# wirrell/SPART-python

Hardware: AMD Instinct MI355X
Metric: SPART spectra/sec (R_TOC+R_TOA+L_TOA) at batch 1M; achieved HBM GB/s vs peak (higher is better)
Workload: dtype f32

## Files before the change

spart-python_amd/build.py:

```python
import hashlib
import os
import subprocess
import sys
import tempfile

HERE = os.path.dirname(os.path.abspath(__file__))
CSRC = os.path.join(HERE, "csrc")
SRC = os.path.join(CSRC, "spart_capi.hip")
SOURCES = [SRC, os.path.join(CSRC, "spart_bands_f32.hip")]
DEPS = SOURCES + [os.path.join(CSRC, f) for f in ("spart_kernels.h", "spart_math.h", "spart_e3_coeffs.h", "spart_f64_tables.h",
                                                  "spart_bands_f32.h", "spart_lut.h")] + [os.path.join(HERE, "..", "include", "spart_hip.h")]
OUT = os.path.join(HERE, "libspart_hip.so")
CFLAGS = ["-O3", "--offload-arch=gfx950", "-std=c++17", "-fPIC", "-fno-slp-vectorize"]
LDFLAGS = ["--offload-arch=gfx950", "-shared", "-fPIC", "-ldl"]
FLAGS = CFLAGS + LDFLAGS
TU_FLAGS = {"spart_bands_f32.hip": ["-mllvm", "-amdgpu-sched-strategy=iterative-minreg"]}


def hipcc():
    for c in (os.environ.get("HIPCC"), "/opt/rocm/bin/hipcc", "hipcc"):
        if c and (os.path.isabs(c) and os.path.exists(c) or not os.path.isabs(c)):
            return c
    return "hipcc"


BUILD_ID_TAG = b"SPART_BUILD_ID:"


def tu_flags(src, extra=()):
    return CFLAGS + TU_FLAGS.get(os.path.basename(src), []) + list(extra)


def source_id(fast_math=True, extra=()):
    h = hashlib.sha256()
    for d in sorted(DEPS, key=os.path.basename):
        h.update(os.path.basename(d).encode() + b"\0")
        h.update(open(d, "rb").read())
    for s in SOURCES:
        h.update((os.path.basename(s) + ":" + " ".join(tu_flags(s, extra))).encode())
    h.update(" ".join(LDFLAGS).encode() + (b"|fast" if fast_math else b"|ieee"))
    return h.hexdigest()[:12]


def binary_id(path=None):
    try:
        data = open(path or OUT, "rb").read()
    except OSError:
        return None
    i = data.find(BUILD_ID_TAG)
    if i < 0:
        return None
    j = i + len(BUILD_ID_TAG)
    return data[j:j + 12].decode("ascii", "replace")


def needs_build(fast_math=True):
    return binary_id() != source_id(fast_math)


def device_asm(outdir, extra=()):
    outs, procs = [], []
    for s in SOURCES:
        o = os.path.join(outdir, os.path.basename(s) + ".s")
        procs.append(subprocess.Popen([hipcc(), *tu_flags(s, extra), "-DSPART_FAST_MATH=1", "-S", "--cuda-device-only", "-o", o, s],
                                      stderr=subprocess.DEVNULL))
        outs.append(o)
    for p in procs:
        if p.wait() != 0:
            raise subprocess.CalledProcessError(p.returncode, p.args)
    return outs


def _compile_and_link(out, defines, extra, verbose):
    with tempfile.TemporaryDirectory(prefix="spart_build_") as tmp:
        objs, procs = [], []
        for s in SOURCES:
            o = os.path.join(tmp, os.path.basename(s) + ".o")
            cmd = [hipcc(), *tu_flags(s, extra), *defines, "-c", "-o", o, s]
            if verbose:
                print("[spart_amd] " + " ".join(cmd), file=sys.stderr, flush=True)
            procs.append((subprocess.Popen(cmd), cmd))
            objs.append(o)
        for p, cmd in procs:
            if p.wait() != 0:
                raise subprocess.CalledProcessError(p.returncode, cmd)
        cmd = [hipcc(), *LDFLAGS, "-o", out, *objs]
        if verbose:
            print("[spart_amd] " + " ".join(cmd), file=sys.stderr, flush=True)
        subprocess.check_call(cmd)


def build(force=False, fast_math=None, verbose=True, out=None, extra=()):
    if out is not None:
        _compile_and_link(out, ["-DSPART_FAST_MATH=1", f'-DSPART_BUILD_ID="{source_id(True, extra)}"'], extra, verbose)
        return out
    if fast_math is None:
        fast_math = os.environ.get("SPART_FAST_MATH", "1") == "1"
    if not force and not needs_build(fast_math):
        return OUT
    tmp = f"{OUT}.tmp.{os.getpid()}"
    defines = [f'-DSPART_BUILD_ID="{source_id(fast_math)}"'] + (["-DSPART_FAST_MATH=1"] if fast_math else [])
    try:
        _compile_and_link(tmp, defines, (), verbose)
        os.replace(tmp, OUT)
    finally:
        if os.path.exists(tmp):
            os.remove(tmp)
    return OUT


if __name__ == "__main__":
    build(force="--force" in sys.argv, fast_math=True if "--fast-math" in sys.argv else None)
    print(OUT)
```

spart-python_amd/csrc/spart_kernels.h:

```cpp
#pragma once

#include "spart_math.h"

namespace spart {

constexpr int TILE = 256;
constexpr int NTILE = 8;
constexpr int NTILE_FULL = 9;
constexpr int MAX_NB = NWLS;

__device__ __forceinline__ void xcd_map(unsigned b, int& tile, int64_t& ck) {
  tile = (int)((b >> 3) & 7u);
  ck = (int64_t)(b >> 6) * 8 + (b & 7u);
}
inline unsigned xcd_grid(int64_t nchunk) { return (unsigned)(((nchunk + 7) / 8) * 64); }

struct ParamPtrs {
  const double* p[NPARAM];
  const double* rho_th;
  const double* tau_th;
  const double* lidf;
  int nlayers;
};

inline int64_t row_pitch_of(int64_t B) { return (B + 63) & ~int64_t(63); }

template <typename T> struct ConstCol {
  const T* p;
  int64_t stride;
  __device__ __forceinline__ T operator[](int i) const { return p[(int64_t)i * stride]; }
};

template <typename T>
__device__ __forceinline__ void stage_constants(T* lds_c, const T* __restrict__ blk, int64_t Bp, int nsub) {
  static_assert(TILE == 256 && NCONST % 8 == 0, "8 rows of 32 samples per pass");
  const int si = threadIdx.x & 31, i0 = threadIdx.x >> 5;
  const unsigned lane_off = ((unsigned)i0 * (unsigned)Bp + (unsigned)si) * (unsigned)sizeof(T);
  if (si < nsub) {
#pragma unroll
    for (int k = 0; k < NCONST / 8; ++k) {
      const T* row = blk + (int64_t)(8 * k) * Bp;
      lds_c[si * NCONST + i0 + 8 * k] = *reinterpret_cast<const T*>(reinterpret_cast<const char*>(row) + lane_off);
    }
  }
}

template <typename T, int SUB>
__device__ __forceinline__ void stage_fetch(T (&r)[NCONST * SUB / TILE], const T* __restrict__ blk, int64_t Bp, int nsub) {
  constexpr int RP = TILE / SUB;
  static_assert(TILE % SUB == 0 && NCONST % RP == 0, "whole passes");
  const int si = threadIdx.x % SUB, i0 = threadIdx.x / SUB;
  const unsigned lane_off = ((unsigned)i0 * (unsigned)Bp + (unsigned)si) * (unsigned)sizeof(T);
  if (si < nsub) {
#pragma unroll
    for (int k = 0; k < NCONST / RP; ++k) {
      const T* row = blk + (int64_t)(RP * k) * Bp;
      r[k] = *reinterpret_cast<const T*>(reinterpret_cast<const char*>(row) + lane_off);
    }
  }
}
template <typename T, int SUB>
__device__ __forceinline__ void stage_put(T* lds_c, const T (&r)[NCONST * SUB / TILE], int nsub) {
  constexpr int RP = TILE / SUB;
  const int si = threadIdx.x % SUB, i0 = threadIdx.x / SUB;
  if (si < nsub) {
#pragma unroll
    for (int k = 0; k < NCONST / RP; ++k) lds_c[si * NCONST + i0 + RP * k] = r[k];
  }
}

struct PreludeStore {
  float* cstF;
  double* cstD;
  double* atm;
  int64_t Bp, s;
  __device__ __forceinline__ void c(int i, double v) const {
    if (cstF) cstF[i * Bp + s] = (float)v;
    if (cstD) cstD[i * Bp + s] = v;
  }
  __device__ __forceinline__ void a(int i, double v) const {
    if (atm) atm[i * Bp + s] = v;
  }
  __device__ __forceinline__ void l(int, double) const {}
};

constexpr int PRELUDE_SIMD_WAVES = 3;
template <bool FAST, bool USER = false>
__global__ __launch_bounds__(256, PRELUDE_SIMD_WAVES) void k_prelude(ParamPtrs pp, int mask, int64_t B, int64_t Bp, float* __restrict__ cstF,
                                                 double* __restrict__ cstD, double* __restrict__ atm) {
  const int64_t base = (int64_t)blockIdx.x * blockDim.x;
  int64_t s = base + threadIdx.x;
  if (!FAST && (mask & PRE_CANOPY) && !(USER && pp.lidf)) {
    constexpr int NB = 32;
    __shared__ int cnt[NB], start[NB];
    __shared__ unsigned char perm[256];
    const int t = threadIdx.x;
    int bucket = NB - 1;
    if (s < B) {
      const double key = ::fabs(pp.p[16][s]) + ::fabs(pp.p[17][s]);
      const double q = key * (NB / 1.0);
      bucket = !(q < (double)(NB - 1)) ? NB - 1 : (q > 0.0 ? (int)q : 0);
    }
    if (t < NB) cnt[t] = 0;
    __syncthreads();
    const int pos = atomicAdd(&cnt[bucket], 1);
    __syncthreads();
    if (t == 0) {
      int acc = 0;
      for (int i = 0; i < NB; ++i) { start[i] = acc; acc += cnt[i]; }
    }
    __syncthreads();
    perm[start[bucket] + pos] = (unsigned char)t;
    __syncthreads();
    s = base + perm[t];
  }
  if (s >= B) return;
  double rho_th = pp.rho_th ? pp.rho_th[s] : 0.01;
  double tau_th = pp.tau_th ? pp.tau_th[s] : 0.01;
  PreludeStore out{cstF, cstD, atm, Bp, s};
  if (USER)
    sample_prelude_to<FAST, true>([&pp, s](int i) { return pp.p[i] ? pp.p[i][s] : 0.0; }, rho_th, tau_th, mask, out,
                                  pp.lidf ? pp.lidf + s * NLINCL : nullptr, pp.nlayers);
  else
    sample_prelude_to<FAST>([&pp, s](int i) { return pp.p[i] ? pp.p[i][s] : 0.0; }, rho_th, tau_th, mask, out);
}

static __global__ __launch_bounds__(256) void k_lidf(const double* __restrict__ a, const double* __restrict__ b, int64_t B,
                                              double* __restrict__ lidf) {
  int64_t s = (int64_t)blockIdx.x * blockDim.x + threadIdx.x;
  if (s >= B) return;
  double li[NLINCL];
  leaf_angles(a[s], b[s], li);
#pragma unroll
  for (int i = 0; i < NLINCL; ++i) lidf[s * NLINCL + i] = li[i];
}

template <typename T> __device__ __forceinline__ BandTab<T> load_tab(const T* __restrict__ tab, int i) {
  BandTab<T> t;
  t.kab = tab[TAB_KAB * NWL + i];
  t.kca = tab[TAB_KCA * NWL + i];
  t.kdm = tab[TAB_KDM * NWL + i];
  t.kw = tab[TAB_KW * NWL + i];
  t.ks = tab[TAB_KS * NWL + i];
  t.kant = tab[TAB_KANT * NWL + i];
  t.kcbc = tab[TAB_CBC * NWL + i];
  t.kprot = tab[TAB_PROT * NWL + i];
  t.talf = tab[TAB_TALF * NWL + i];
  t.t12 = tab[TAB_T12 * NWL + i];
  t.t21 = tab[TAB_T21 * NWL + i];
  t.g0 = tab[TAB_GSV0 * NWL + i];
  t.g1 = tab[TAB_GSV1 * NWL + i];
  t.g2 = tab[TAB_GSV2 * NWL + i];
  t.cbac = tab[TAB_CBAC * NWL + i];
  t.pw = tab[TAB_PW * NWL + i];
  t.rw = tab[TAB_RW * NWL + i];
  return t;
}

template <typename T, typename C> __device__ __forceinline__ CanopyPar<T> load_canopy(const C& c) {
  CanopyPar<T> cp;
  cp.sob = c[C_SOB]; cp.sof = c[C_SOF];
  cp.hbf = c[C_HBF]; cp.ks = c[C_KS]; cp.ko = c[C_KO]; cp.lai = c[C_LAI]; cp.lai2 = c[C_LAI2];
  cp.tss = c[C_TSS]; cp.too = c[C_TOO]; cp.Z = c[C_Z]; cp.hot = c[C_HOT]; cp.pso2w = c[C_PSO2W];
  return cp;
}

template <bool NT = false, typename T> __device__ __forceinline__ void store_row(T* row, unsigned byte_off, T v) {
  T* p = reinterpret_cast<T*>(reinterpret_cast<char*>(row) + byte_off);
  if (NT) __builtin_nontemporal_store(v, p);
  else *p = v;
}
inline bool nt_ok(int pitch_elems, size_t elem_size) { return ((size_t)pitch_elems * elem_size) % 128 == 0; }

template <typename T> struct MatPtrs {
  T *leaf_refl, *leaf_tran, *leaf_kchl, *soil_refl, *soil_dry, *rso, *rdo, *rsd, *rdd;
  const T* rdry_in;
  int pf, po;
};

template <typename T, int MAT, int FULL, bool NT = false>
__global__ __launch_bounds__(TILE, (sizeof(T) == 8 ? 3 : 1))
void k_bands(const T* __restrict__ tab, const T* __restrict__ cst, int64_t Bp, int64_t B, int chunk, MatPtrs<T> mat,
             T* __restrict__ bandsum) {
  int tile;
  int64_t ck;
  xcd_map(blockIdx.x, tile, ck);
  if (ck * chunk >= B) return;
  if (sizeof(T) == 8) stage_f64_tables();
  const int band = tile * TILE + threadIdx.x;
  const bool active = band < NEVAL;
  const bool thermal = band == NWL;
  const int ti = band < NWL ? band : NWL - 1;
  const BandTab<T> tb = load_tab(tab, ti);
  const int64_t s0 = ck * chunk;
  const int64_t s1 = (s0 + chunk < B) ? s0 + chunk : B;
  T sum_so = T(0), sum_do = T(0), sum_sd = T(0), sum_dd = T(0);
  unsigned off_f = (unsigned)band * (unsigned)sizeof(T), off_o = off_f;
  if (MAT) {
    const int64_t b0f = s0 * mat.pf, b0o = s0 * mat.po;
    if (mat.leaf_refl) mat.leaf_refl += b0f;
    if (mat.leaf_tran) mat.leaf_tran += b0f;
    if (mat.soil_refl) mat.soil_refl += b0f;
    if (mat.rso) mat.rso += b0f;
    if (mat.rdo) mat.rdo += b0f;
    if (mat.rsd) mat.rsd += b0f;
    if (mat.rdd) mat.rdd += b0f;
    if (mat.leaf_kchl) mat.leaf_kchl += b0o;
    if (mat.soil_dry) mat.soil_dry += b0o;
  }
  constexpr int SUB = 32;
  constexpr bool HOIST_FILM = sizeof(T) == 8;
  constexpr bool PINGPONG = sizeof(T) == 4 && MAT == 0;
  __shared__ __attribute__((aligned(16))) T lds_all[(PINGPONG ? 2 : 1) * SUB * NCONST];
  T stg[NCONST * SUB / TILE];
  int cur = 0;
  if (PINGPONG) {
    const int n0 = (int)((s1 - s0 < SUB) ? (s1 - s0) : SUB);
    stage_fetch<T, SUB>(stg, cst + s0, Bp, n0);
    stage_put<T, SUB>(lds_all, stg, n0);
    __syncthreads();
  }
  for (int64_t sb = s0; sb < s1; sb += SUB) {
  const int nsub = (int)((s1 - sb < SUB) ? (s1 - sb) : SUB);
  T* const lds_c = lds_all + cur * (SUB * NCONST);
  const int nnext = (int)((s1 - sb - SUB < SUB) ? (s1 - sb - SUB) : SUB);
  if (PINGPONG) {
    if (nnext > 0) stage_fetch<T, SUB>(stg, cst + sb + SUB, Bp, nnext);
  } else {
    __syncthreads();
    stage_constants<T>(lds_c, cst + sb, Bp, nsub);
    __syncthreads();
  }
  bool film_same = false;
  T tw1s = T(0);
  if (HOIST_FILM) {
    const int l = threadIdx.x & 63;
    const T f0 = lds_c[C_FILM2L];
    const T fl = lds_c[(l < nsub ? l : 0) * NCONST + C_FILM2L];
    film_same = __all(fl == f0) != 0;
    if (film_same) tw1s = soil_tw1<T>(tb, f0);
  }
  constexpr bool AHEAD = MAT == 0 && sizeof(T) == 4;
  T lc[9];
#pragma unroll
  for (int i = 0; i < 9; ++i) lc[i] = lds_c[i];
  for (int si = 0; si < nsub; ++si) {
    const int64_t s = sb + si;
    const T* c = lds_c + si * NCONST;
    T refl, tran, absb, K;
    static_assert(C_CAB == 0 && C_NM1 == 8, "lc[] = constants 0..8 in leaf_band's argument order");
    if (!AHEAD) {
#pragma unroll
      for (int i = 0; i < 9; ++i) lc[i] = c[i];
    }
    leaf_band<T>(tb, lc[0], lc[1], lc[2], lc[3], lc[4], lc[5], lc[6], lc[7], lc[8], refl, tran, absb, K);
    if (AHEAD) {
      const T* cn = lds_c + ((si + 1 < nsub) ? si + 1 : si) * NCONST;
#pragma unroll
      for (int i = 0; i < 9; ++i) lc[i] = cn[i];
    }
    T rho = refl, tau = tran, ab = absb;
    if (tile == NTILE - 1) {
      rho = thermal ? c[C_RHO_TH] : refl;
      tau = thermal ? c[C_TAU_TH] : tran;
      ab = thermal ? (T(1) - c[C_RHO_TH] - c[C_TAU_TH]) : absb;
    }
    if (MAT && active) {
      if (mat.leaf_refl) store_row<NT>(mat.leaf_refl, off_f, rho);
      if (mat.leaf_tran) store_row<NT>(mat.leaf_tran, off_f, tau);
      if (!thermal && mat.leaf_kchl) store_row<NT>(mat.leaf_kchl, off_o, (K > T(0)) ? divx(c[C_CAB] * tb.kab, K) : T(0));
    }
    const CanopyPar<T> cp = load_canopy<T>(c);
    const CanopyCore<T> core = canopy_core_l<T>(cp, rho, tau, ab, c[C_KSL], c[C_KOL]);
    T rdry = (MAT == 2) ? mat.rdry_in[s * mat.po + ti] : soil_dry<T>(tb, c[C_F1], c[C_F2], c[C_F3]);
    T fm[7] = {c[C_FM0], c[C_FM1], c[C_FM2], c[C_FM3], c[C_FM4], c[C_FM5], c[C_FM6]};
    T rwet;
    if (HOIST_FILM) {
      const T tw1 = film_same ? tw1s : soil_tw1<T>(tb, c[C_FILM2L]);
      soil_band_tw<T>(tb, rdry, c[C_WET], fm, c[C_FMSUM], tw1, rwet);
    } else {
      soil_band<T>(tb, rdry, c[C_WET], fm, c[C_FMSUM], c[C_FILM2L], rwet);
    }
    if (MAT && active) {
      if (mat.soil_refl) store_row<NT>(mat.soil_refl, off_f, rwet);
      if (!thermal && mat.soil_dry) store_row<NT>(mat.soil_dry, off_o, rdry);
    }
    constexpr bool SUM_ONLY = FULL == 1 && MAT == 0 && sizeof(T) == 4;
    T rso, rdo, rsd, rdd;
    if (SUM_ONLY) {
      sum_so += canopy_soil_sum<T>(cp, core, rwet, c[C_TSTO]);
    } else {
      canopy_soil<T>(cp, core, rwet, rso, rdo, rsd, rdd);
      if (FULL == 2) {
        sum_so += rso; sum_do += rdo; sum_sd += rsd; sum_dd += rdd;
      } else if (FULL == 1) {
        sum_so += (rso + rdo) + (rsd + rdd);
      }
    }
    if (MAT) {
      if (active) {
        if (mat.rso) store_row<NT>(mat.rso, off_f, rso);
        if (mat.rdo) store_row<NT>(mat.rdo, off_f, rdo);
        if (mat.rsd) store_row<NT>(mat.rsd, off_f, rsd);
        if (mat.rdd) store_row<NT>(mat.rdd, off_f, rdd);
      }
      constexpr int TH_WAVE = (NWL % TILE) / 64, TH_LANE = (NWL % TILE) % 64;
      if (tile == NTILE - 1 && (int)(threadIdx.x >> 6) == TH_WAVE) {
        const unsigned pad = off_f + (unsigned)((TH_LANE + 1) * (int)sizeof(T));
        T* arrs[7] = {mat.leaf_refl, mat.leaf_tran, mat.soil_refl, mat.rso, mat.rdo, mat.rsd, mat.rdd};
        const T vals[7] = {rho, tau, rwet, rso, rdo, rsd, rdd};
        const int l = threadIdx.x & 63;
#pragma unroll
        for (int q = 0; q < 7; ++q) {
          const T v = __shfl(vals[q], TH_LANE, 64);
          if (arrs[q]) {
            store_row(arrs[q], pad, v);
            store_row(arrs[q], pad + 64u * (unsigned)sizeof(T), v);
            if (l < NWLT - 1 - 128) store_row(arrs[q], pad + 128u * (unsigned)sizeof(T), v);
          }
        }
      }
      off_f += (unsigned)mat.pf * (unsigned)sizeof(T);
      off_o += (unsigned)mat.po * (unsigned)sizeof(T);
    }
  }
  if (PINGPONG) {
    if (nnext > 0) stage_put<T, SUB>(lds_all + (cur ^ 1) * (SUB * NCONST), stg, nnext);
    __syncthreads();
    cur ^= 1;
  }
  }
  if (FULL == 2) {
    T* bs = bandsum + (ck * (NTILE * TILE) + band) * 4;
    bs[0] = sum_so; bs[1] = sum_do; bs[2] = sum_sd; bs[3] = sum_dd;
  } else if (FULL == 1) {
    bandsum[ck * (NTILE * TILE) + band] = sum_so;
  }
}

template <typename T> struct LdsCol {
  const T* p;
  __device__ __forceinline__ T operator[](int i) const { return p[i * 64]; }
};


constexpr int COL_WAVES = 4;
constexpr int COLUMNS_SIMD_WAVES = 4;

template <typename TG, typename TO, typename TR>
__global__ __launch_bounds__(64 * COL_WAVES, COLUMNS_SIMD_WAVES) void k_columns(
    const TG* __restrict__ tab, const TG* __restrict__ cst, const double* __restrict__ atm, int64_t Bp,
    const int* __restrict__ band0, const int* __restrict__ band1, const double* __restrict__ frac,
    const double* __restrict__ coef, const double* __restrict__ econv, int nb, const TR* __restrict__ rdry_in, int po, int64_t B,
    TO* __restrict__ R_TOC, TO* __restrict__ R_TOA, TO* __restrict__ L_TOA, TO* __restrict__ o_rsoil, TO* __restrict__ o_La) {
  __shared__ TG lds_c[NCONST_USED * 64];
  __shared__ double lds_a[NATM_USED * 64];
  __shared__ double lds_k[COL_WAVES * 64];
  if (sizeof(TG) == 8) stage_f64_tables();
  const int lane = threadIdx.x & 63;
  const int wave = __builtin_amdgcn_readfirstlane((int)(threadIdx.x >> 6));
  const int64_t s0 = (int64_t)blockIdx.x * 64;
  const int64_t s = s0 + lane;
  const bool ok = s < B;
  const int64_t sc = ok ? s : B - 1;
  for (int i = wave; i < NCONST_USED; i += COL_WAVES) lds_c[i * 64 + lane] = cst[(int64_t)i * Bp + sc];
  for (int i = wave; i < NATM_USED; i += COL_WAVES) lds_a[i * 64 + lane] = atm[(int64_t)i * Bp + sc];
  __syncthreads();
  const LdsCol<TG> c{lds_c + lane};
  const LdsCol<double> a{lds_a + lane};
  const bool want_soil = o_rsoil != nullptr;
  for (int j = wave; j < nb; j += COL_WAVES) {
    const int b0 = band0[j], b1 = band1[j];
    const double f = frac[j];
    const double kv = coef[(size_t)(lane < NCOEF ? lane : NCOEF - 1) * nb + j];
    double y0[5], y1[5];
#pragma unroll 1
    for (int e = 0; e < 2; ++e) {
      if (e == 1 && b1 == b0) break;
      const int band = e ? b1 : b0;
      const bool thermal = band == NWL;
      const int ti = band < NWL ? band : NWL - 1;
      const BandTab<TG> tb = load_tab(tab, ti);
      TG refl, tran, absb, K;
      leaf_band<TG>(tb, c[C_CAB], c[C_CCA], c[C_CDM], c[C_CW], c[C_CS], c[C_CANT], c[C_CBC], c[C_PROT], c[C_NM1], refl,
                    tran, absb, K);
      const TG rho = thermal ? c[C_RHO_TH] : refl;
      const TG tau = thermal ? c[C_TAU_TH] : tran;
      const TG ab = thermal ? (TG(1) - c[C_RHO_TH] - c[C_TAU_TH]) : absb;
      const CanopyPar<TG> cp = load_canopy<TG>(c);
      const CanopyCore<TG> core = canopy_core<TG>(cp, rho, tau, ab);
      const TG rdry = rdry_in ? (TG)rdry_in[sc * po + ti] : soil_dry<TG>(tb, c[C_F1], c[C_F2], c[C_F3]);
      TG fm[7] = {c[C_FM0], c[C_FM1], c[C_FM2], c[C_FM3], c[C_FM4], c[C_FM5], c[C_FM6]};
      TG rwet;
      soil_band<TG>(tb, rdry, c[C_WET], fm, c[C_FMSUM], c[C_FILM2L], rwet);
      TG rso, rdo, rsd, rdd;
      canopy_soil<TG>(cp, core, rwet, rso, rdo, rsd, rdd);
      const double v[5] = {(double)rso, (double)rdo, (double)rsd, (double)rdd, (double)rwet};
#pragma unroll
      for (int q = 0; q < 5; ++q) {
        if (e == 0) y0[q] = v[q];
        y1[q] = v[q];
      }
    }
    double v[5];
#pragma unroll
    for (int q = 0; q < 5; ++q) v[q] = y0[q] + (y1[q] - y0[q]) * f;
    double* kw = lds_k + wave * 64;
    kw[lane] = kv;
    __builtin_amdgcn_fence(__ATOMIC_RELEASE, "wavefront");
    __builtin_amdgcn_wave_barrier();
    __builtin_amdgcn_fence(__ATOMIC_ACQUIRE, "wavefront");
    const SmacOut so = smac_band_c(a, [kw](int r) { return kw[r]; });
    const double La = a[A_LAF] * econv[j];
    double rtoc, rtoa, ltoa;
    toc_to_toa(so, v[0], v[1], v[3], v[2], La, rtoc, rtoa, ltoa);
    if (ok) {
      const int64_t o = s * nb + j;
      R_TOC[o] = (TO)rtoc;
      R_TOA[o] = (TO)rtoa;
      L_TOA[o] = (TO)ltoa;
      if (want_soil) o_rsoil[o] = (TO)v[4];
      if (o_La) o_La[o] = (TO)La;
    }
  }
}

template <typename T>
__global__ __launch_bounds__(256) void k_bandmean(const T* __restrict__ bandsum, int64_t nchunk, int64_t B,
                                                  T* __restrict__ out) {
  int i = blockIdx.x * blockDim.x + threadIdx.x;
  if (i >= 4 * NWLS) return;
  int q = i / NWLS, band = i % NWLS;
  int ev = band < NWL ? band : NWL;
  double acc = 0.0;
  for (int64_t c = 0; c < nchunk; ++c) acc += (double)bandsum[(c * (NTILE * TILE) + ev) * 4 + q];
  out[i] = (T)(acc / (double)B);
}

template <typename T, bool STAGE, typename F>
__device__ __forceinline__ void for_samples_staged(const T* __restrict__ cst, int64_t Bp, int64_t s0, int64_t s1, F&& body) {
  if (!STAGE) {
    for (int64_t s = s0; s < s1; ++s) body(s, ConstCol<T>{cst + s, Bp});
    return;
  }
  constexpr int SUB = 32;
  __shared__ __attribute__((aligned(16))) T lds_c[SUB * NCONST];
  for (int64_t sb = s0; sb < s1; sb += SUB) {
    const int nsub = (int)((s1 - sb < SUB) ? (s1 - sb) : SUB);
    __syncthreads();
    stage_constants<T>(lds_c, cst + sb, Bp, nsub);
    __syncthreads();
    for (int si = 0; si < nsub; ++si) body(sb + si, (const T*)(lds_c + si * NCONST));
  }
}

template <typename T, bool NT>
__global__ __launch_bounds__(TILE) void k_prospect(const T* __restrict__ tab, const T* __restrict__ cst, int64_t Bp, int64_t B,
                                                   int chunk, int po, T* __restrict__ o_refl,
                                                   T* __restrict__ o_tran, T* __restrict__ o_kchl) {
  int tile;
  int64_t ck;
  xcd_map(blockIdx.x, tile, ck);
  if (ck * chunk >= B) return;
  if (sizeof(T) == 8) stage_f64_tables();
  const int band = tile * TILE + threadIdx.x;
  const bool active = band < NWL;
  const BandTab<T> tb = load_tab(tab, active ? band : NWL - 1);
  const int64_t s0 = ck * chunk;
  const int64_t s1 = (s0 + chunk < B) ? s0 + chunk : B;
  unsigned off = (unsigned)band * (unsigned)sizeof(T);
  if (o_refl) o_refl += s0 * po;
  if (o_tran) o_tran += s0 * po;
  if (o_kchl) o_kchl += s0 * po;
  for_samples_staged<T, sizeof(T) == 4>(cst, Bp, s0, s1, [&](int64_t, auto c) {
    T refl, tran, absb, K;
    leaf_band<T>(tb, c[C_CAB], c[C_CCA], c[C_CDM], c[C_CW], c[C_CS], c[C_CANT], c[C_CBC], c[C_PROT], c[C_NM1], refl,
                 tran, absb, K);
// ... 113 lines not shown
```

spart-python_amd/csrc/spart_math.h:

```cpp
#pragma once

#include <cmath>
#include <cstdint>

#if defined(__HIPCC__)
#include <hip/hip_runtime.h>
#define SPART_HD __host__ __device__ __forceinline__
#else
#define SPART_HD inline
#endif

#if defined(__clang__)
#define SPART_NO_CONTRACT _Pragma("clang fp contract(off)")
#else
#define SPART_NO_CONTRACT
#endif

#if defined(__HIP_DEVICE_COMPILE__)
#define SPART_WAVE_ANY(c) (__builtin_amdgcn_ballot_w64(c) != 0)
#define SPART_KEEP_BRANCH(x) asm volatile("" : "+v"(x))
#else
#define SPART_WAVE_ANY(c) (c)
#define SPART_KEEP_BRANCH(x) ((void)0)
#endif
// ... 163 lines not shown
template <> struct Mx<double> {
  static SPART_HD double horner_c(double p, double x, double c) {
#if defined(__HIPCC__)
    return spart_horner(p, x, c);
#else
    return p * x + c;
#endif
  }
#if defined(__HIP_DEVICE_COMPILE__) && defined(SPART_FAST_MATH)
  static SPART_HD double exp_poly(double x) {
    x = (x < -800.0) ? -800.0 : x;
    const double k = __builtin_rint(x * 1.4426950408889634);
    double r = __builtin_fma(-k, 6.93147180369123816490e-01, x);
    r = __builtin_fma(-k, 1.90821492927058770002e-10, r);
    spart_cdp ce = spart_fresh(c_EXP_F64);
    double p = ce[11];
#pragma unroll
    for (int i = 10; i >= 0; --i) p = spart_horner(p, r, ce[i]);
    p = __builtin_fma(p * r, r, r);
    return __builtin_ldexp(1.0 + p, (int)k);
  }
  static SPART_HD double exp_finish(double k, double r) {
    const int ki = (int)k;
    const double t = s_f64_exp_tab[ki & (F64_EXP_TAB - 1)];
    double p = spart_horner(1.0 / 24.0, r, 1.0 / 6.0);
    p = __builtin_fma(p, r, 0.5);
    p = __builtin_fma(p, r * r, r);
    return __builtin_ldexp(__builtin_fma(t, p, t), ki >> 8);
  }
  static SPART_HD double exp(double x) {
    x = __builtin_fmax(x, -800.0);
    const double k = __builtin_rint(x * 369.32993046757463);
    double r = __builtin_fma(-k, 0.0027076061737716373, x);
    r = __builtin_fma(-k, 2.9064910585985925e-13, r);
    return exp_finish(k, r);
  }
  static SPART_HD double exp2(double x) {
    const double t = x * 256.0;
    const double k = __builtin_rint(t);
    return exp_finish(k, (t - k) * 0.0027076061740622863);
  }
  static SPART_HD double log(double x) {
    const unsigned long long u = (unsigned long long)__double_as_longlong(x);
    const unsigned hi = (unsigned)(u >> 32);
    const int e = (int)(hi >> 20) - 1023;
    const unsigned i = (hi >> 12) & (unsigned)(F64_LOG_TAB - 1);
    const double m = __longlong_as_double((long long)((u & 0x000FFFFFFFFFFFFFull) | 0x3FF0000000000000ull));
    const double R = s_f64_log_tab[2 * i], L = s_f64_log_tab[2 * i + 1];
    const double z = __builtin_fma(m, R, -1.0);
    double q = spart_horner(-1.0 / 6.0, z, 0.2);
    q = spart_horner(q, z, -0.25);
    q = spart_horner(q, z, 1.0 / 3.0);
    q = __builtin_fma(q, z, -0.5);
    const double p = __builtin_fma(z * z, q, z);
    return __builtin_fma((double)e, 0.6931471805599453, L + p);
  }
#else
  static SPART_HD double exp_poly(double x) { return ::exp(x); }
  static SPART_HD double exp(double x) { return ::exp(x); }
  static SPART_HD double exp2(double x) { return ::exp2(x); }
  static SPART_HD double log(double x) { return ::log(x); }
#endif
  static SPART_HD double sqrt(double x) {
#if defined(__HIP_DEVICE_COMPILE__) && defined(SPART_FAST_MATH)
    const double y0 = __builtin_amdgcn_rsq(x + 1e-300);
    const double g = x * y0;
    const double e = __builtin_fma(-g, y0, 1.0);
    return __builtin_fma(g * 0.5, e, g);
#else
    return ::sqrt(x);
#endif
  }
  static SPART_HD double rcp(double x) {
#if defined(__HIP_DEVICE_COMPILE__) && defined(SPART_FAST_MATH)
    const double r = __builtin_amdgcn_rcp(x);
    return __builtin_fma(__builtin_fma(-x, r, 1.0), r, r);
#else
    return 1.0 / x;
#endif
  }
  static SPART_HD double log1p(double x) {
#if defined(SPART_FAST_MATH)
    if (x < 0.1) {
      double s = x * rcp(2.0 + x), s2 = s * s;
      double p = horner_c(1.0 / 13.0, s2, 1.0 / 11.0);
      p = horner_c(p, s2, 1.0 / 9.0);
      p = horner_c(p, s2, 1.0 / 7.0);
      p = horner_c(p, s2, 0.2);
      p = horner_c(p, s2, 1.0 / 3.0);
      p = p * s2 + 1.0;
      return 2.0 * s * p;
    }
    return log(1.0 + x);
#else
    return ::log1p(x);
#endif
  }
  static SPART_HD double omen_taylor(double z) {
    double p = -1.0 / 40320.0;
    p = p * z + 1.0 / 5040.0;
    p = p * z - 1.0 / 720.0;
    p = p * z + 1.0 / 120.0;
    p = p * z - 1.0 / 24.0;
    p = p * z + 1.0 / 6.0;
    p = p * z - 0.5;
    p = p * z + 1.0;
    return z * p;
  }
  static SPART_HD double one_minus_exp_neg(double z) {
#if defined(SPART_FAST_MATH)
    if (::fabs(z) < 0.02) return omen_taylor(z);
    return 1.0 - exp(-z);
#else
    return -::expm1(-z);
#endif
  }
  static SPART_HD double one_minus_exp_neg_poly(double z) {
#if defined(SPART_FAST_MATH)
    return (::fabs(z) < 0.02) ? omen_taylor(z) : 1.0 - exp_poly(-z);
#else
    return -::expm1(-z);
#endif
  }
  static SPART_HD double one_minus_exp_neg(double z, double ez) {
#if defined(SPART_FAST_MATH)
    return (::fabs(z) < 0.02) ? omen_taylor(z) : 1.0 - ez;
#else
    (void)ez;
    return -::expm1(-z);
#endif
  }
  static SPART_HD double fabs(double x) { return ::fabs(x); }
  static SPART_HD double fmax(double a, double b) { return ::fmax(a, b); }
  static SPART_HD double tiny() { return 1e-300; }
};

template <typename T> SPART_HD T divx(T a, T b) { return a * Mx<T>::rcp(b); }

template <typename T> struct SailJ;
template <> struct SailJ<float> {
  static constexpr float THRESH = 0.06f;
  static SPART_HD float poly(float d) {
    return 1.0f + d * (-0.5f + d * (0.166666667f + d * (-0.0416666667f + d * 8.33333333e-3f)));
  }
};
template <> struct SailJ<double> {
  static constexpr double THRESH = 2e-3;
  static SPART_HD double poly(double d) {
    return 1.0 + d * (-0.5 + d * (1.0 / 6.0 + d * (-1.0 / 24.0 + d * (1.0 / 120.0 - d * (1.0 / 720.0)))));
  }
};
template <typename T> SPART_HD T sail_j1_d(T L, T tk, T e1, T d, T id) {
  T v = L * (tk - e1) * id;
  const bool small = Mx<T>::fabs(d) < SailJ<T>::THRESH;
  if (SPART_WAVE_ANY(small)) {
    SPART_KEEP_BRANCH(d);
    v = small ? L * tk * SailJ<T>::poly(d) : v;
  }
  return v;
}
template <typename T> SPART_HD T sail_j2_d(T L, T tk, T e1, T kpm, T ikpm) {
  T d = kpm * L;
  T v = (T(1) - tk * e1) * ikpm;
  if (SPART_WAVE_ANY(d < SailJ<T>::THRESH)) {
    SPART_KEEP_BRANCH(d);
    v = (d < SailJ<T>::THRESH) ? L * SailJ<T>::poly(d) : v;
  }
  return v;
}

template <typename T> struct E3c;
template <> struct E3c<float> {
  static constexpr int GD = E3_G_DEG_F32, WD = E3_W_DEG_F32;
  static constexpr float PSCALE = 2.0f;
  static SPART_HD const float* gt() { return E3_G_F32; }
  static SPART_HD const float* pt() { return E3_P_F32; }
  static SPART_HD const float* qt() { return E3_Q_F32; }
};
#if defined(__HIPCC__)
static_assert(E3_G_DEG_F64 == 12 && E3_W_DEG_F64 == 6, "tables below list the coefficients one by one");
#define SPART_L13(a) {a[0], a[1], a[2], a[3], a[4], a[5], a[6], a[7], a[8], a[9], a[10], a[11], a[12]}
#define SPART_L7(a) {a[0], a[1], a[2], a[3], a[4], a[5], a[6]}
static __device__ __constant__ double c_E3_G_F64[13] = SPART_L13(E3_G_F64);
#define SPART_L7X2(a) {2 * a[0], 2 * a[1], 2 * a[2], 2 * a[3], 2 * a[4], 2 * a[5], 2 * a[6]}
static __device__ __constant__ double c_E3_P_F64[7] = SPART_L7X2(E3_P_F64);
static __device__ __constant__ double c_E3_Q_F64[7] = SPART_L7(E3_Q_F64);
#endif
template <> struct E3c<double> {
  static constexpr int GD = E3_G_DEG_F64, WD = E3_W_DEG_F64;
#if defined(__HIP_DEVICE_COMPILE__)
  static constexpr double PSCALE = 1.0;
#else
  static constexpr double PSCALE = 2.0;
#endif
#if defined(__HIP_DEVICE_COMPILE__)
  static SPART_HD spart_cdp gt() { return spart_fresh(c_E3_G_F64); }
  static SPART_HD spart_cdp pt() { return spart_fresh(c_E3_P_F64); }
  static SPART_HD spart_cdp qt() { return spart_fresh(c_E3_Q_F64); }
#else
  static SPART_HD const double* gt() { return E3_G_F64; }
  static SPART_HD const double* pt() { return E3_P_F64; }
  static SPART_HD const double* qt() { return E3_Q_F64; }
#endif
};

#if defined(__HIPCC__)
SPART_HD double horner_uniform(double p, double x, double c) { return spart_horner(p, x, c); }
#else
SPART_HD double horner_uniform(double p, double x, double c) { return p * x + c; }
#endif
SPART_HD float horner_uniform(float p, float x, float c) { return p * x + c; }

template <typename T> SPART_HD void plate_tau(T K, T& tau, T& u) {
  using C = E3c<T>;
  T x = (K < Mx<T>::tiny()) ? Mx<T>::tiny() : K;
  const bool small = x < T(1);
  T tl, ul;
  if (small) {
    const auto cg = C::gt();
    T g = cg[C::GD];
#pragma unroll
    for (int i = C::GD - 1; i >= 0; --i) g = horner_uniform(g, x, cg[i]);
    ul = x * (g + x * Mx<T>::log(x));
    tl = T(1) - ul;
  } else {
    const auto cp = C::pt(), cq = C::qt();
    T pn = C::PSCALE * cp[0], qn = cq[0];
#pragma unroll
    for (int i = 1; i <= C::WD; ++i) {
      pn = horner_uniform(pn, x, C::PSCALE * cp[i]);
      qn = horner_uniform(qn, x, cq[i]);
    }
    tl = Mx<T>::exp(-x) * pn * Mx<T>::rcp((x + T(3)) * qn);
    ul = T(1) - tl;
  }
  tau = tl;
  u = ul;
}

inline double calculate_tav(double alpha, double nr) {
  const double rd = PI / 180.0;
  double n2 = nr * nr, n_p = n2 + 1, nm = n2 - 1;
  double a = (nr + 1) * (nr + 1) / 2;
  double k = -(n2 - 1) * (n2 - 1) / 4;
  double sa = std::sin(alpha * rd);
  double b1 = 0;
  if (alpha != 90) b1 = std::sqrt((sa * sa - n_p / 2) * (sa * sa - n_p / 2) + k);
  double b2 = sa * sa - n_p / 2;
  double b = b1 - b2;
  double b3 = b * b * b, a3 = a * a * a;
  double ts = (k * k / (6 * b3) + k / b - b / 2) - (k * k / (6 * a3) + k / a - a / 2);
  double tp1 = -2 * n2 * (b - a) / (n_p * n_p);
  double tp2 = -2 * n2 * n_p * std::log(b / a) / (nm * nm);
  double tp3 = n2 * (1 / b - 1 / a) / 2;
  double tp4 = 16 * n2 * n2 * (n2 * n2 + 1) * std::log((2 * n_p * b - nm * nm) / (2 * n_p * a - nm * nm)) /
               (n_p * n_p * n_p * nm * nm);
  double tp5 = 16 * n2 * n2 * n2 * (1 / (2 * n_p * b - nm * nm) - 1 / (2 * n_p * a - nm * nm)) / (n_p * n_p * n_p);
  double tp = tp1 + tp2 + tp3 + tp4 + tp5;
  return (ts + tp) / (2 * sa * sa);
}

inline double wl_solar_at(int i) {
  return i < NWL ? 400.0 + i : (i < NWL + 126 ? 2500.0 + 100.0 * (i - NWL) : 16000.0 + 1000.0 * (i - NWL - 126));
}

inline void interp_support(double x, int& e0, int& e1, double& frac) {
  auto eval_of = [](int grid_idx) { return grid_idx < NWL ? grid_idx : NWL; };
  int i0 = 0;
  while (i0 + 1 < NWLS - 1 && wl_solar_at(i0 + 1) <= x) ++i0;
  int i1 = i0 + 1;
  double f = (x - wl_solar_at(i0)) / (wl_solar_at(i1) - wl_solar_at(i0));
  if (!(f > 0.0)) f = 0.0;
  if (f > 1.0) f = 1.0;
  e0 = eval_of(i0);
  e1 = f > 0.0 ? eval_of(i1) : e0;
  frac = f;
}

enum TabRow {
  TAB_KAB = 0, TAB_KCA, TAB_KDM, TAB_KW, TAB_KS, TAB_KANT, TAB_CBC, TAB_PROT,
  TAB_TALF, TAB_T12, TAB_T21,
  TAB_GSV0, TAB_GSV1, TAB_GSV2,
  TAB_CBAC, TAB_PW, TAB_RW,
  NTAB
};

template <typename T> struct BandTab {
  T kab, kca, kdm, kw, ks, kant, kcbc, kprot, talf, t12, t21, g0, g1, g2, cbac, pw, rw;
};

enum ConstIdx {
  C_CAB = 0, C_CCA, C_CDM, C_CW, C_CS, C_CANT, C_CBC, C_PROT, C_NM1, C_RHO_TH, C_TAU_TH,
  C_F1, C_F2, C_F3, C_WET, C_FM0, C_FM1, C_FM2, C_FM3, C_FM4, C_FM5, C_FM6, C_FMSUM, C_FILM2L,
  C_SOB, C_SOF, C_HBF, C_KS, C_KO, C_LAI, C_LAI2, C_TSS, C_TOO, C_Z, C_HOT, C_PSO2W,
  C_KSL, C_KOL, C_TSTO, C_RSV3,
  NCONST
};
constexpr int NCONST_USED = C_KSL;
static_assert(NCONST == 40, "constant block is 40 values");

enum AtmIdx {
  A_US = 0, A_UV, A_M, A_PEQ, A_PA, A_AOT, A_CKSI, A_KSID, A_LAF,
  A_LOGPEQ, A_LOGM, A_LOGO3M, A_LOGH2OM,
  A_RSV,
  NATM = 16
};
constexpr int NATM_USED = A_RSV;

template <typename T>
SPART_HD void leaf_band(const BandTab<T>& tb, T cab, T cca, T cdm, T cw, T cs, T cant, T cbc, T prot, T nm1,
                        T& refl, T& tran, T& absb, T& Kall) {
  T K = cab * tb.kab + cca * tb.kca + cdm * tb.kdm + cw * tb.kw + cs * tb.ks + cant * tb.kant + cbc * tb.kcbc +
        prot * tb.kprot;
  Kall = K;
  T tau, u;
  plate_tau(K, tau, u);
  T r21 = T(1) - tb.t21, r12 = T(1) - tb.t12, ralf = T(1) - tb.talf;
  T x = r21 * tau;
  T inv = Mx<T>::rcp(T(1) - x * x);
  T Ta, t;
  if constexpr (sizeof(T) == 4) {
    T ti = tau * inv;
    Ta = (tb.talf * tb.t21) * ti;
    t = (tb.t12 * tb.t21) * ti;
  } else {
    T c = tau * tb.t21 * inv;
    Ta = tb.talf * c;
    t = tb.t12 * c;
  }
  T Ra = ralf + x * Ta;
  T r = r12 + x * t;
  T gq = u * (T(1) + x) * inv;
  T a1 = tb.t12 * gq;
  T atop = tb.talf * gq;
  T tt = Mx<T>::fmax(t, Mx<T>::tiny());
  T D = Mx<T>::sqrt((T(1) + r + tt) * (T(1) + r - tt) * (T(1) - r + tt) * a1);
  T i2rt = Mx<T>::rcp(T(2) * r * tt);
  T am1 = (a1 * (T(1) - r + tt) + D) * (tt * i2rt);
  T bm1 = (a1 * (T(1) - tt + r) + D) * (r * i2rt);
  T a = T(1) + am1;
  T sq, omsq;
  if constexpr (sizeof(T) == 4) {
    T z2 = nm1 * Mx<T>::log2_1p(bm1);
    sq = Mx<T>::exp2(-z2);
    omsq = Mx<T>::one_minus_exp2_neg(z2, sq);
  } else {
    T z = nm1 * Mx<T>::log1p(bm1);
    sq = Mx<T>::exp(-z);
    omsq = Mx<T>::one_minus_exp_neg(z, sq);
  }
  T omq = omsq * (T(1) + sq);
  T A2 = am1 * (a + T(1));
  T aomq = a * omq;
  T iE = Mx<T>::rcp(A2 + omq - aomq * r);
  T TaE = Ta * iE;
  tran = TaE * sq * A2;
  refl = Ra + TaE * aomq * t;
  absb = atop + TaE * (am1 * omsq * (a - sq) + aomq * a1);
}

template <typename T> SPART_HD T soil_tw1(const BandTab<T>& tb, T film2l) { return Mx<T>::exp2(-film2l * tb.kw); }

template <typename T>
SPART_HD void soil_band_tw(const BandTab<T>& tb, T rdry, T wet, const T fm[7], T fmsum16, T tw1, T& rwet) {
  if constexpr (sizeof(T) == 4) {
    const T cb = T(1) - tb.cbac;
    T rbac = rdry * (cb * (T(1) - rdry) + T(1));
    T xv = rbac * tw1;
    T D = T(1) - tb.pw * xv;
    T N = fm[1] * xv;
#pragma unroll
    for (int k = 1; k < 6; ++k) {
      xv *= tw1;
      const T d = T(1) - tb.pw * xv;
      N = N * d + fm[k + 1] * xv * D;
      D *= d;
    }
    T v = rdry * fm[0] + tb.rw * fmsum16 + (T(1) - tb.rw) * (T(1) - tb.pw) * N * Mx<T>::rcp(D);
    rwet = (wet > T(0)) ? v : rdry;
    return;
  }
  T rbac = T(1) - (T(1) - rdry) * (rdry * tb.cbac + T(1) - rdry);
  T x[6], d[6], pre[6];
  T xv = rbac;
#pragma unroll
  for (int k = 0; k < 6; ++k) {
    xv *= tw1;
    x[k] = xv;
    d[k] = T(1) - tb.pw * xv;
    pre[k] = (k == 0) ? d[0] : pre[k - 1] * d[k];
  }
  T q = Mx<T>::rcp(pre[5]);
  T acc = T(0);
#pragma unroll
  for (int k = 5; k >= 1; --k) {
    acc += fm[k + 1] * x[k] * (q * pre[k - 1]);
    q *= d[k];
  }
  acc += fm[1] * x[0] * q;
  T v = rdry * fm[0] + tb.rw * fmsum16 + (T(1) - tb.rw) * (T(1) - tb.pw) * acc;
  rwet = (wet > T(0)) ? v : rdry;
}
template <typename T>
SPART_HD void soil_band(const BandTab<T>& tb, T rdry, T wet, const T fm[7], T fmsum16, T film2l, T& rwet) {
  soil_band_tw<T>(tb, rdry, wet, fm, fmsum16, soil_tw1<T>(tb, film2l), rwet);
}

template <typename T> SPART_HD T soil_dry(const BandTab<T>& tb, T f1, T f2, T f3) {
  return f1 * tb.g0 + f2 * tb.g1 + f3 * tb.g2;
}

template <typename T> struct CanopyPar {
  T sob, sof, hbf, ks, ko, lai, lai2, tss, too, Z, hot, pso2w;
};

template <typename T> struct CanopyCore {
  T rho_so, rho_dd, tau_dd, tau_sd, tau_do, rho_sd, rho_do;
};

template <typename T>
SPART_HD CanopyCore<T> canopy_core_l(const CanopyPar<T>& c, T rho, T tau, T absb, T ksl, T kol) {
  T P = T(0.5) * (rho + tau);
  T Mn = c.hbf * (rho - tau);
  T sigb = P + Mn;
  T w = c.sob * rho + c.sof * tau;
  T a = T(1) - P + Mn;
  T m = Mx<T>::sqrt(absb * (T(1) + T(2) * Mn));
  T apm = a + m, ksm = c.ks + m, kom = c.ko + m;
  T kk = ksm * kom;
  T i3 = Mx<T>::rcp(apm * kk);
  T iam = i3 * kk;
  T ikk = i3 * apm;
  T iks = ikk * kom, iko = ikk * ksm;
  T rinf = sigb * iam;
  T rinf2 = rinf * rinf;
  T omr = (absb + m) * iam;
  T opr = T(1) + rinf;
  T omr2 = omr * opr;
  T L = c.lai;
  T e1 = Mx<T>::exp2(-m * c.lai2);
  const T thr = SailJ<T>::THRESH;
  T d1, d2;
  if constexpr (sizeof(T) == 4) {
    d1 = m * L - ksl;
    d2 = m * L - kol;
  } else {
    (void)ksl, (void)kol;
    d1 = (m - c.ks) * L;
    d2 = (m - c.ko) * L;
  }
  T d1s = (Mx<T>::fabs(d1) < thr) ? T(1) : d1, d2s = (Mx<T>::fabs(d2) < thr) ? T(1) : d2;
  T idd = Mx<T>::rcp(d1s * d2s);
  T J1k = sail_j1_d<T>(L, c.tss, e1, d1, idd * d2s);
  T J1K = sail_j1_d<T>(L, c.too, e1, d2, idd * d1s);
  T J2k = sail_j2_d<T>(L, c.tss, e1, ksm, iks);
  T J2K = sail_j2_d<T>(L, c.too, e1, kom, iko);
  T ome2 = T(1) - e1 * e1;
  T re = rinf * e1;
  T i1 = Mx<T>::rcp(omr2 * (T(1) + rinf2));
  T i2 = (T(1) + rinf2) * i1;
  T U = P * opr, V = Mn * omr;
  T s1 = c.ks * U - V;
  T s2 = c.ks * U + V;
  T v1 = c.ko * U - V;
  T v2 = c.ko * U + V;
  T Pss = s1 * J1k, Qss = s2 * J2k, Poo = v1 * J1K, Qoo = v2 * J2K;
  T tau_dd = omr2 * e1 * i1;
  T rho_dd = rinf * ome2 * i1;
  T tau_sd = (Pss - re * Qss) * i1;
  T tau_do = (Poo - re * Qoo) * i1;
  T rho_sd = (Qss - re * Pss) * i1;
  T rho_do = (Qoo - re * Poo) * i1;
  T T1 = v2 * s1 * (c.Z - J1k * c.too) * iko + v1 * s2 * (c.Z - J1K * c.tss) * iks;
  T T2 = -(Qoo * rho_sd + Poo * tau_sd) * rinf;
  T rho_sod = (T1 + T2) * i2;
  T rho_so = rho_sod + w * c.hot;
  return CanopyCore<T>{rho_so, rho_dd, tau_dd, tau_sd, tau_do, rho_sd, rho_do};
}

template <typename T> SPART_HD CanopyCore<T> canopy_core(const CanopyPar<T>& c, T rho, T tau, T absb) {
  return canopy_core_l<T>(c, rho, tau, absb, c.ks * c.lai, c.ko * c.lai);
}

template <typename T>
SPART_HD void canopy_soil(const CanopyPar<T>& c, const CanopyCore<T>& k, T rs, T& rso, T& rdo, T& rsd, T& rdd) {
  const T rho_so = k.rho_so, rho_dd = k.rho_dd, tau_dd = k.tau_dd, tau_sd = k.tau_sd, tau_do = k.tau_do, rho_sd = k.rho_sd,
          rho_do = k.rho_do;
  T g = rs * Mx<T>::rcp(T(1) - rs * rho_dd);
  T h = g * tau_dd;
  T tst = c.tss + tau_sd;
  rso = rho_so + rs * c.pso2w + ((tau_sd + c.tss * rs * rho_dd) * c.too + tst * tau_do) * g;
  rdo = rho_do + (c.too + tau_do) * h;
  rsd = rho_sd + tst * h;
  rdd = rho_dd + tau_dd * h;
}

template <typename T> SPART_HD T canopy_soil_sum(const CanopyPar<T>& c, const CanopyCore<T>& k, T rs, T tsto) {
  T q = rs * k.rho_dd;
  T g = rs * Mx<T>::rcp(T(1) - q);
  T tdo = c.too + k.tau_do;
  T inner = k.tau_sd * tdo + c.tss * k.tau_do + tsto * q + k.tau_dd * ((c.tss + k.tau_sd) + tdo + k.tau_dd);
  return ((k.rho_so + k.rho_do) + (k.rho_sd + k.rho_dd)) + rs * c.pso2w + g * inner;
}

template <typename T>
SPART_HD void canopy_band(const CanopyPar<T>& c, T rho, T tau, T absb, T rs, T& rso, T& rdo, T& rsd, T& rdd) {
  const CanopyCore<T> k = canopy_core<T>(c, rho, tau, absb);
  canopy_soil<T>(c, k, rs, rso, rdo, rsd, rdd);
}


SPART_HD double lidf_dcum(double a, double b, double theta_deg) {
  const double rd = PI / 180.0;
  if (a > 1.0) return 1.0 - ::cos(theta_deg * rd);
  double x = 2.0 * rd * theta_deg;
  const double theta2 = x;
  double y = 0.0, dx;
  int it = 0;
  do {
    double sn, cs;
    ::sincos(x, &sn, &cs);
    y = sn * (a + b * cs);
    dx = 0.5 * (y - x + theta2);
    x += dx;
  } while (::fabs(dx) > 1e-8 && ++it < 100000);
  return (2.0 * y + theta2) / PI;
}

SPART_HD double lidf_theta(int i);
SPART_HD double lidf_sin_2theta(int i);
SPART_HD double lidf_cos_2theta(int i);
SPART_HD void lidf_sincos(double u, double s2, double c2, double& sn, double& cs);
SPART_HD double lidf_dcum_newton(double a, double b, int i) {
  const double theta_deg = lidf_theta(i);
  if (!(::fabs(a) + ::fabs(b) < 0.95)) return lidf_dcum(a, b, theta_deg);
  const double rd = PI / 180.0;
  const double theta2 = 2.0 * rd * theta_deg;
  const double s2 = lidf_sin_2theta(i), c2 = lidf_cos_2theta(i);
  double y = s2 * (a + b * c2);
  for (int it = 0; it < 12; ++it) {
    double sn, cs;
    lidf_sincos(y, s2, c2, sn, cs);
    const double f = y - sn * (a + b * cs);
    const double fp = 1.0 - a * cs - b * (2.0 * cs * cs - 1.0);
    const double d = f / fp;
    y -= d;
    if (::fabs(d) < 1e-9) break;
  }
  return (2.0 * y + theta2) / PI;
}

SPART_HD double lidf_theta(int i) { return (i < 8) ? 10.0 * (i + 1) : 80.0 + 2.0 * (i - 7); }
SPART_HD double lidf_litab(int i) { return (i < 8) ? 5.0 + 10.0 * i : 81.0 + 2.0 * (i - 8); }

SPART_HD void lidf_sincos(double u, double s2, double c2, double& sn, double& cs) {
  const double u2 = u * u;
  double ps = -1.0 / 121645100408832000.0;
  ps = ps * u2 + 1.0 / 355687428096000.0;
  ps = ps * u2 - 1.0 / 1307674368000.0;
  ps = ps * u2 + 1.0 / 6227020800.0;
  ps = ps * u2 - 1.0 / 39916800.0;
  ps = ps * u2 + 1.0 / 362880.0;
  ps = ps * u2 - 1.0 / 5040.0;
  ps = ps * u2 + 1.0 / 120.0;
  ps = ps * u2 - 1.0 / 6.0;
  ps = ps * u2 + 1.0;
  double pc = 1.0 / 6402373705728000.0;
  pc = pc * u2 - 1.0 / 20922789888000.0;
  pc = pc * u2 + 1.0 / 87178291200.0;
  pc = pc * u2 - 1.0 / 479001600.0;
  pc = pc * u2 + 1.0 / 3628800.0;
  pc = pc * u2 - 1.0 / 40320.0;
  pc = pc * u2 + 1.0 / 720.0;
  pc = pc * u2 - 1.0 / 24.0;
  pc = pc * u2 + 0.5;
  const double su = u * ps, cu = 1.0 - u2 * pc;
  sn = s2 * cu + c2 * su;
  cs = c2 * cu - s2 * su;
}
SPART_HD void lidf_rotate(double d, double& sn, double& cs) {
  const double d2 = d * d;
  double ps = -1.0 / 39916800.0;
  ps = ps * d2 + 1.0 / 362880.0;
  ps = ps * d2 - 1.0 / 5040.0;
  ps = ps * d2 + 1.0 / 120.0;
  ps = ps * d2 - 1.0 / 6.0;
  const double sd = d + d * (d2 * ps);
  double pc = -1.0 / 479001600.0;
  pc = pc * d2 + 1.0 / 3628800.0;
  pc = pc * d2 - 1.0 / 40320.0;
  pc = pc * d2 + 1.0 / 720.0;
  pc = pc * d2 - 1.0 / 24.0;
  pc = pc * d2 + 0.5;
  const double cm = d2 * pc;
  const double s0 = sn, c0 = cs;
  sn = s0 + (c0 * sd - s0 * cm);
  cs = c0 - (s0 * sd + c0 * cm);
}
constexpr double LIDF_ROT_MAX = 0.25;
SPART_HD void lidf_sincos_step(bool rot, double d, double u_new, double s2, double c2, double& sn, double& cs) {
  double sr = sn, cr = cs;
  if (SPART_WAVE_ANY(rot)) lidf_rotate(d, sr, cr);
  if (SPART_WAVE_ANY(!rot)) {
    double sf, cf;
    lidf_sincos(u_new, s2, c2, sf, cf);
    sr = rot ? sr : sf;
    cr = rot ? cr : cf;
  }
  sn = sr;
  cs = cr;
}

template <bool JUMP> SPART_HD double lidf_dcum_lit_impl(double a, double b, int i, int* jumped = nullptr) {
  if (!(::fabs(a) + 0.5 * ::fabs(b) <= 1.0)) return lidf_dcum(a, b, lidf_theta(i));
  const double rd = PI / 180.0;
  const double theta2 = 2.0 * rd * lidf_theta(i);
  const double s2 = lidf_sin_2theta(i), c2 = lidf_cos_2theta(i);
  constexpr double LIDF_KJUMP = 2e-2;
  constexpr double LIDF_GATE = 1e-2;
  const double kjump = LIDF_KJUMP / (0.25 * (::fabs(a) + 2.0 * ::fabs(b)) + 0.02);
  double u = 0.0, y, dx = 0.0, dprev;
  double sn = s2, cs = c2;
  bool more, ready = false;
  int it = 0;
  do {
    dprev = dx;
    u += dx;
    lidf_sincos_step((it & 7) != 7 && ::fabs(dx) < LIDF_ROT_MAX, dx, u, s2, c2, sn, cs);
    y = sn * (a + b * cs);
    dx = 0.5 * (y - u);
    more = ::fabs(dx) > 1e-8;
    if (JUMP && ::fabs(dx) < LIDF_GATE) {
      const double ad = ::fabs(dx), ap = ::fabs(dprev), df = ap - ad;
      ready = dx * dprev > 0.0 && ad > 0.3 * ap && ad < 0.98 * ap && ap * ap * ap < kjump * (df * df);
    }
  } while (more && !ready && ++it < 100000);
  if (JUMP && more && ready) {
    using Md = Mx<double>;
    const double d0 = dx * dprev * Md::rcp(dprev - dx);
    double us = u + d0;
    double nstep = 1.0;
    lidf_sincos_step(::fabs(d0) < LIDF_ROT_MAX, d0, us, s2, c2, sn, cs);
    for (int k = 0; k < 3; ++k) {
      const double f = sn * (a + b * cs) - us;
      const double fp = a * cs + b * (2.0 * cs * cs - 1.0) - 1.0;
      nstep = f * Md::rcp(fp);
      us -= nstep;
      lidf_sincos_step(::fabs(nstep) < LIDF_ROT_MAX, -nstep, us, s2, c2, sn, cs);
    }
    const double s2x = 2.0 * sn * cs, c2x = 2.0 * cs * cs - 1.0;
    const double y1 = a * cs + b * c2x, y2 = -a * sn - 2.0 * b * s2x, y3 = -a * cs - 4.0 * b * c2x, y4 = a * sn + 8.0 * b * s2x;
    const double r = 0.5 * (1.0 + y1), q2 = 0.25 * y2, q3 = y3 * (1.0 / 12.0), q4 = y4 * (1.0 / 48.0);
    const double r2 = r * r;
    const double i1 = Md::rcp(r - r2);
    const double a2 = q2 * i1;
// ... 473 lines not shown
```

Baseline: 95.69 million.

## Add wave-uniform fast path and algebraic simplifications to f32 band kernel

```diff
diff --git a/spart-python_amd/build.py b/spart-python_amd/build.py
--- a/spart-python_amd/build.py
+++ b/spart-python_amd/build.py
@@ -14,7 +14,7 @@
 CFLAGS = ["-O3", "--offload-arch=gfx950", "-std=c++17", "-fPIC", "-fno-slp-vectorize"]
 LDFLAGS = ["--offload-arch=gfx950", "-shared", "-fPIC", "-ldl"]
 FLAGS = CFLAGS + LDFLAGS
-TU_FLAGS = {"spart_bands_f32.hip": ["-mllvm", "-amdgpu-sched-strategy=iterative-minreg"]}
+TU_FLAGS = {"spart_bands_f32.hip": []}
 
 
 def hipcc():
diff --git a/spart-python_amd/csrc/spart_kernels.h b/spart-python_amd/csrc/spart_kernels.h
--- a/spart-python_amd/csrc/spart_kernels.h
+++ b/spart-python_amd/csrc/spart_kernels.h
@@ -1,4 +1,6 @@
 #pragma once
+
+#include <type_traits>
 
 #include "spart_math.h"
 
@@ -244,6 +246,17 @@
   T lc[9];
 #pragma unroll
   for (int i = 0; i < 9; ++i) lc[i] = lds_c[i];
+  constexpr bool COMMON = sizeof(T) == 4 && MAT == 0 && FULL == 1;
+  bool common = false;
+  T tw1c = T(0);
+  if (COMMON) {
+    const int l = threadIdx.x & 63;
+    const T* cl = lds_c + (l < nsub ? l : 0) * NCONST;
+    common = __all(cl[C_FILM2L] == lds_c[C_FILM2L] && cl[C_CBC] == T(0) && cl[C_PROT] == T(0)) != 0;
+    if (common) tw1c = soil_tw1<T>(tb, lds_c[C_FILM2L]);
+  }
+  auto sample_loop = [&](auto common_tag) __attribute__((always_inline)) {
+  constexpr bool FAST = decltype(common_tag)::value;
   for (int si = 0; si < nsub; ++si) {
     const int64_t s = sb + si;
     const T* c = lds_c + si * NCONST;
@@ -253,7 +266,7 @@
 #pragma unroll
       for (int i = 0; i < 9; ++i) lc[i] = c[i];
     }
-    leaf_band<T>(tb, lc[0], lc[1], lc[2], lc[3], lc[4], lc[5], lc[6], lc[7], lc[8], refl, tran, absb, K);
+    leaf_band<T, !FAST>(tb, lc[0], lc[1], lc[2], lc[3], lc[4], lc[5], lc[6], lc[7], lc[8], refl, tran, absb, K);
     if (AHEAD) {
       const T* cn = lds_c + ((si + 1 < nsub) ? si + 1 : si) * NCONST;
 #pragma unroll
@@ -275,7 +288,9 @@
     T rdry = (MAT == 2) ? mat.rdry_in[s * mat.po + ti] : soil_dry<T>(tb, c[C_F1], c[C_F2], c[C_F3]);
     T fm[7] = {c[C_FM0], c[C_FM1], c[C_FM2], c[C_FM3], c[C_FM4], c[C_FM5], c[C_FM6]};
     T rwet;
-    if (HOIST_FILM) {
+    if (FAST) {
+      soil_band_tw<T>(tb, rdry, c[C_WET], fm, c[C_FMSUM], tw1c, rwet);
+    } else if (HOIST_FILM) {
       const T tw1 = film_same ? tw1s : soil_tw1<T>(tb, c[C_FILM2L]);
       soil_band_tw<T>(tb, rdry, c[C_WET], fm, c[C_FMSUM], tw1, rwet);
     } else {
@@ -323,6 +338,13 @@
       off_f += (unsigned)mat.pf * (unsigned)sizeof(T);
       off_o += (unsigned)mat.po * (unsigned)sizeof(T);
     }
+  }
+  };
+  if constexpr (COMMON) {
+    if (common) sample_loop(std::true_type{});
+    else sample_loop(std::false_type{});
+  } else {
+    sample_loop(std::false_type{});
   }
   if (PINGPONG) {
     if (nnext > 0) stage_put<T, SUB>(lds_all + (cur ^ 1) * (SUB * NCONST), stg, nnext);
diff --git a/spart-python_amd/csrc/spart_math.h b/spart-python_amd/csrc/spart_math.h
--- a/spart-python_amd/csrc/spart_math.h
+++ b/spart-python_amd/csrc/spart_math.h
@@ -339,6 +339,15 @@
 };
 template <typename T> SPART_HD T sail_j1_d(T L, T tk, T e1, T d, T id) {
   T v = L * (tk - e1) * id;
+  const bool small = Mx<T>::fabs(d) < SailJ<T>::THRESH;
+  if (SPART_WAVE_ANY(small)) {
+    SPART_KEEP_BRANCH(d);
+    v = small ? L * tk * SailJ<T>::poly(d) : v;
+  }
+  return v;
+}
+template <typename T> SPART_HD T sail_j1_a(T L, T tk, T e1, T d, T ia) {
+  T v = L * Mx<T>::fabs(tk - e1) * ia;
   const bool small = Mx<T>::fabs(d) < SailJ<T>::THRESH;
   if (SPART_WAVE_ANY(small)) {
     SPART_KEEP_BRANCH(d);
@@ -494,11 +503,12 @@
 };
 constexpr int NATM_USED = A_RSV;
 
-template <typename T>
+template <typename T, bool PRO = true>
 SPART_HD void leaf_band(const BandTab<T>& tb, T cab, T cca, T cdm, T cw, T cs, T cant, T cbc, T prot, T nm1,
                         T& refl, T& tran, T& absb, T& Kall) {
-  T K = cab * tb.kab + cca * tb.kca + cdm * tb.kdm + cw * tb.kw + cs * tb.ks + cant * tb.kant + cbc * tb.kcbc +
-        prot * tb.kprot;
+  T K = cab * tb.kab + cca * tb.kca + cdm * tb.kdm + cw * tb.kw + cs * tb.ks + cant * tb.kant;
+  if (PRO) K = K + cbc * tb.kcbc + prot * tb.kprot;
+  else (void)cbc, (void)prot;
   Kall = K;
   T tau, u;
   plate_tau(K, tau, u);
@@ -517,14 +527,16 @@
   }
   T Ra = ralf + x * Ta;
   T r = r12 + x * t;
-  T gq = u * (T(1) + x) * inv;
+  T gq;
+  if constexpr (sizeof(T) == 4) gq = u * __builtin_fmaf(x, inv, inv);
+  else gq = u * (T(1) + x) * inv;
   T a1 = tb.t12 * gq;
   T atop = tb.talf * gq;
   T tt = Mx<T>::fmax(t, Mx<T>::tiny());
   T D = Mx<T>::sqrt((T(1) + r + tt) * (T(1) + r - tt) * (T(1) - r + tt) * a1);
   T i2rt = Mx<T>::rcp(T(2) * r * tt);
   T am1 = (a1 * (T(1) - r + tt) + D) * (tt * i2rt);
-  T bm1 = (a1 * (T(1) - tt + r) + D) * (r * i2rt);
+  T bm1 = (a1 * (sizeof(T) == 4 ? T(1) + r - tt : T(1) - tt + r) + D) * (r * i2rt);
   T a = T(1) + am1;
   T sq, omsq;
   if constexpr (sizeof(T) == 4) {
@@ -552,18 +564,19 @@
 SPART_HD void soil_band_tw(const BandTab<T>& tb, T rdry, T wet, const T fm[7], T fmsum16, T tw1, T& rwet) {
   if constexpr (sizeof(T) == 4) {
     const T cb = T(1) - tb.cbac;
+    const T c2 = (T(1) - tb.rw) * (T(1) - tb.pw) * Mx<T>::rcp(tb.pw);
     T rbac = rdry * (cb * (T(1) - rdry) + T(1));
-    T xv = rbac * tw1;
-    T D = T(1) - tb.pw * xv;
-    T N = fm[1] * xv;
+    T y = rbac * (tb.pw * tw1);
+    T D = T(1) - y;
+    T N = fm[1];
 #pragma unroll
     for (int k = 1; k < 6; ++k) {
-      xv *= tw1;
-      const T d = T(1) - tb.pw * xv;
-      N = N * d + fm[k + 1] * xv * D;
+      y *= tw1;
+      const T d = T(1) - y;
+      N = N * d + fm[k + 1] * D;
       D *= d;
     }
-    T v = rdry * fm[0] + tb.rw * fmsum16 + (T(1) - tb.rw) * (T(1) - tb.pw) * N * Mx<T>::rcp(D);
+    T v = rdry * fm[0] + tb.rw * fmsum16 + c2 * (N * Mx<T>::rcp(D) - fmsum16);
     rwet = (wet > T(0)) ? v : rdry;
     return;
   }
@@ -636,10 +649,18 @@
     d1 = (m - c.ks) * L;
     d2 = (m - c.ko) * L;
   }
-  T d1s = (Mx<T>::fabs(d1) < thr) ? T(1) : d1, d2s = (Mx<T>::fabs(d2) < thr) ? T(1) : d2;
-  T idd = Mx<T>::rcp(d1s * d2s);
-  T J1k = sail_j1_d<T>(L, c.tss, e1, d1, idd * d2s);
-  T J1K = sail_j1_d<T>(L, c.too, e1, d2, idd * d1s);
+  T J1k, J1K;
+  if constexpr (sizeof(T) == 4) {
+    T d1a = Mx<T>::fmax(Mx<T>::fabs(d1), thr), d2a = Mx<T>::fmax(Mx<T>::fabs(d2), thr);
+    T idd = Mx<T>::rcp(d1a * d2a);
+    J1k = sail_j1_a<T>(L, c.tss, e1, d1, idd * d2a);
+    J1K = sail_j1_a<T>(L, c.too, e1, d2, idd * d1a);
+  } else {
+    T d1s = (Mx<T>::fabs(d1) < thr) ? T(1) : d1, d2s = (Mx<T>::fabs(d2) < thr) ? T(1) : d2;
+    T idd = Mx<T>::rcp(d1s * d2s);
+    J1k = sail_j1_d<T>(L, c.tss, e1, d1, idd * d2s);
+    J1K = sail_j1_d<T>(L, c.too, e1, d2, idd * d1s);
+  }
   T J2k = sail_j2_d<T>(L, c.tss, e1, ksm, iks);
   T J2K = sail_j2_d<T>(L, c.too, e1, kom, iko);
   T ome2 = T(1) - e1 * e1;
@@ -684,10 +705,10 @@
 
 template <typename T> SPART_HD T canopy_soil_sum(const CanopyPar<T>& c, const CanopyCore<T>& k, T rs, T tsto) {
   T q = rs * k.rho_dd;
-  T g = rs * Mx<T>::rcp(T(1) - q);
+  T iq = Mx<T>::rcp(T(1) - q);
   T tdo = c.too + k.tau_do;
   T inner = k.tau_sd * tdo + c.tss * k.tau_do + tsto * q + k.tau_dd * ((c.tss + k.tau_sd) + tdo + k.tau_dd);
-  return ((k.rho_so + k.rho_do) + (k.rho_sd + k.rho_dd)) + rs * c.pso2w + g * inner;
+  return ((k.rho_so + k.rho_do) + (k.rho_sd + k.rho_dd)) + rs * (c.pso2w + inner * iq);
 }
 
 template <typename T>
```

New measurement: 102.7 million (median of 6 runs). 7.3% higher.
